# gau-nernst/llama-x

Measured on NVIDIA B200. Metric: train tokens/s, Llama-3.1-8B INT8+LoRA prefix-LM, higher is better.
Workload: dtype int8 fwd (int32 acc) / bf16 bwd

## Files before the change

include/llamax_b200.h:

```cpp
#ifndef LLAMAX_B200_H_
#define LLAMAX_B200_H_

#include <stdint.h>

#ifdef __cplusplus
extern "C" {
#endif

#define LLAMAX_B200_VERSION 102

#define LLAMAX_OK 0
#define LLAMAX_ERR_ARG (-1)
#define LLAMAX_ERR_CUDA (-2)

const char* llamax_last_error(void);
int llamax_version(void);
int llamax_set_device(int device);
int llamax_set_gemm_cta_group(int cg);

typedef struct {
  const void* lora_h;
  int64_t ldh;
  const void* lora_b;
  int32_t lora_rank;
  float lora_scale;
  const void* resid;
  int64_t ldr;
  int32_t seg_n0, seg_n1;
  const void* rope;
  int32_t rope_S, rope_cols;
} llamax_epilogue_t;

int llamax_int8_gemm_dequant(const void* A, int64_t lda, const void* B, int64_t ldb, const void* a_scale,
                             const void* b_scale, void* C, int64_t ldc, int64_t M, int64_t N, int64_t K,
                             const llamax_epilogue_t* epi, void* stream);
int llamax_int8_gemm_s32(const void* A, int64_t lda, const void* B, int64_t ldb, void* C, int64_t ldc, int64_t M,
                         int64_t N, int64_t K, void* stream);

int llamax_bf16_gemm(const void* A, int64_t lda, const void* B, int64_t ldb, void* C, int64_t ldc, int64_t M,
                     int64_t N, int64_t K, const void* col_scale, int round_before_scale,
                     const llamax_epilogue_t* epi, void* stream);
int llamax_bf16_gemm_swiglu_bwd(const void* A, int64_t lda, const void* B, int64_t ldb, int64_t M, int64_t N, int64_t K,
                                const llamax_epilogue_t* epi, const void* ab, int64_t ld_ab, void* dab, int64_t ld_dab,
                                void* g, void* stream);
int llamax_bf16_gemm_rowdot(const void* A, int64_t lda, const void* B, int64_t ldb, void* C, int64_t ldc, int64_t M,
                            int64_t N, int64_t K, const llamax_epilogue_t* epi, const void* other, int64_t ld_other,
                            void* dot_out, int64_t S, void* stream);

int llamax_bf16_int8_gemm(const void* A, int64_t lda, const void* B8, int64_t ldb8, const void* b_scale, int b_layout,
                          const void* tail, int64_t ldt, void* C, int64_t ldc, int64_t M, int64_t N, int64_t K,
                          int64_t K1, const llamax_epilogue_t* epi, void* stream);
int llamax_bf16_int8_gemm_swiglu_bwd(const void* A, int64_t lda, const void* B8, int64_t ldb8, const void* k_scale,
                                     int64_t M, int64_t N, int64_t K, const llamax_epilogue_t* epi, const void* ab,
                                     int64_t ld_ab, void* dab, int64_t ld_dab, void* g, void* stream);
int llamax_bf16_gemm_tn(const void* At, int64_t ldat, const void* Bt, int64_t ldbt, void* C, int64_t ldc, int64_t M,
                        int64_t N, int64_t K, void* stream);

int llamax_dequant_weight(const void* w8, const void* scale, void* out, int64_t ldo, int64_t N, int64_t K,
                          int transpose, int apply_scale, void* stream);

int llamax_rowquant_int8(const void* x, int64_t ldx, void* q8, void* scale_out, int64_t M, int64_t K,
                         void* stream);
int llamax_rowquant_int8_colscale(const void* x, int64_t ldx, const void* col_scale, void* q8, void* scale_out,
                                  int64_t M, int64_t K, void* stream);

int llamax_rmsnorm_fwd(const void* x, const void* w, void* y, void* rstd, void* q8, void* qscale, int64_t M,
                       int64_t D, float eps, void* stream);
int llamax_rmsnorm_bwd(const void* dy, const void* x, const void* w, const void* rstd, const void* dres, void* dx,
                       void* dw_partial, int32_t nparts, int64_t M, int64_t D, void* stream);
int llamax_reduce_partials(const void* partial, void* out, int32_t nparts, int64_t D, void* stream);

int llamax_swiglu_fwd(const void* a, const void* b, int64_t ld, void* g, void* q8, void* qscale, int64_t M,
                      int64_t F, void* stream);
int llamax_swiglu_bwd(const void* dg, const void* a, const void* b, int64_t ld, void* da, void* db, int64_t ldd,
                      void* g, int64_t M, int64_t F, void* stream);

int llamax_rope_inplace(void* x, int64_t ld, const void* rope, int64_t B, int64_t S, int32_t nheads, int32_t D,
                        int inverse, void* stream);

int llamax_attn_fwd(const void* q, int64_t ldq, const void* k, int64_t ldk, const void* v, int64_t ldv, void* o,
                    int64_t ldo, void* lse, int64_t B, int64_t S, int32_t Hq, int32_t Hkv, int32_t D,
                    int64_t prefix_len, const void* prefix_len_b, const void* doc_start, float scale, void* stream);
int llamax_attn_bwd(const void* q, int64_t ldq, const void* k, int64_t ldk, const void* v, int64_t ldv,
                    const void* o, int64_t ldo, const void* lse, const void* dout, int64_t lddo, void* dq,
                    int64_t lddq, void* dk, int64_t lddk, void* dv, int64_t lddv, void* dq_accum, void* delta,
                    int64_t B, int64_t S, int32_t Hq, int32_t Hkv, int32_t D, int64_t prefix_len,
                    const void* prefix_len_b, const void* doc_start, const void* doc_end, float scale,
                    const void* rope_inverse, void* stream);

int llamax_gelu_bias_fwd(void* z, const void* bias, void* y, int64_t rows, int64_t C, int32_t period, int32_t lo,
                         int32_t hi, void* stream);
int llamax_gelu_bwd(const void* dy, const void* z, void* dz, int64_t rows, int64_t C, int32_t period, int32_t lo,
                    int32_t hi, void* stream);
int llamax_conv_s2k3_col2im(const void* dcol, void* dxp, int64_t B, int64_t Tp, int64_t C, void* stream);

#define LLAMAX_MAX_COPY_JOBS 64
typedef struct {
  const void* src;
  void* dst;
  int64_t src_ld;
  int64_t dst_ld;
  int32_t rows, cols;
  float scale;
  int32_t flags;
} llamax_copy_job_t;
int llamax_batched_copy(const llamax_copy_job_t* jobs, int32_t n_jobs, void* stream);

int llamax_lora_wgrad(const void* X, int64_t ldx, const void* Ht, int64_t ldht, void* out, int64_t M, int64_t P,
                      int32_t R, float alpha, void* stream);

int llamax_lora_bwd_pair(const void* dY, int64_t lddy, const void* Bt, int64_t ldbt, const void* Ht, int64_t ldht,
                         void* dh, int64_t lddh, void* dht, int64_t lddht, void* dh_accum, void* dB, int64_t M,
                         int64_t N, int32_t R, float alpha, void* stream);


int llamax_cross_entropy(void* logits, int64_t ld, const void* labels, void* loss_sum, const void* inv_n, int64_t M,
                         int64_t V, int write_grad, void* stream);

#ifdef __cplusplus
}
#endif
#endif
```

llamax_b200/_lib.py:

```python

import ctypes
import os
import threading
from ctypes import POINTER, Structure, c_char_p, c_float, c_int, c_int32, c_int64, c_void_p

_HERE = os.path.dirname(os.path.abspath(__file__))
LIB_PATH = os.environ.get("LLAMAX_B200_LIB") or os.path.join(_HERE, "csrc", "libllamax_b200.so")

P = c_void_p
I64 = c_int64
I32 = c_int32


class Epilogue(Structure):

    _fields_ = [
        ("lora_h", P),
        ("ldh", I64),
        ("lora_b", P),
        ("lora_rank", I32),
        ("lora_scale", c_float),
        ("resid", P),
        ("ldr", I64),
        ("seg_n0", I32),
        ("seg_n1", I32),
        ("rope", P),
        ("rope_S", I32),
        ("rope_cols", I32),
    ]


EP = POINTER(Epilogue)

MAX_COPY_JOBS = 64


class CopyJob(Structure):

    _fields_ = [
        ("src", P),
        ("dst", P),
        ("src_ld", I64),
        ("dst_ld", I64),
        ("rows", I32),
        ("cols", I32),
        ("scale", c_float),
        ("flags", I32),
    ]

SIGNATURES = {
    "llamax_version": [],
    "llamax_set_device": [c_int],
    "llamax_set_gemm_cta_group": [c_int],
    "llamax_int8_gemm_dequant": [P, I64, P, I64, P, P, P, I64, I64, I64, I64, EP, P],
    "llamax_int8_gemm_s32": [P, I64, P, I64, P, I64, I64, I64, I64, P],
    "llamax_bf16_gemm": [P, I64, P, I64, P, I64, I64, I64, I64, P, c_int, EP, P],
    "llamax_bf16_gemm_swiglu_bwd": [P, I64, P, I64, I64, I64, I64, EP, P, I64, P, I64, P, P],
    "llamax_bf16_gemm_tn": [P, I64, P, I64, P, I64, I64, I64, I64, P],
    "llamax_bf16_gemm_rowdot": [P, I64, P, I64, P, I64, I64, I64, I64, EP, P, I64, P, I64, P],
    "llamax_bf16_int8_gemm": [P, I64, P, I64, P, c_int, P, I64, P, I64, I64, I64, I64, I64, EP, P],
    "llamax_bf16_int8_gemm_swiglu_bwd": [P, I64, P, I64, P, I64, I64, I64, EP, P, I64, P, I64, P, P],
    "llamax_dequant_weight": [P, P, P, I64, I64, I64, c_int, c_int, P],
    "llamax_rowquant_int8": [P, I64, P, P, I64, I64, P],
    "llamax_rowquant_int8_colscale": [P, I64, P, P, P, I64, I64, P],
    "llamax_rmsnorm_fwd": [P, P, P, P, P, P, I64, I64, c_float, P],
    "llamax_rmsnorm_bwd": [P, P, P, P, P, P, P, I32, I64, I64, P],
    "llamax_reduce_partials": [P, P, I32, I64, P],
    "llamax_swiglu_fwd": [P, P, I64, P, P, P, I64, I64, P],
    "llamax_swiglu_bwd": [P, P, P, I64, P, P, I64, P, I64, I64, P],
    "llamax_rope_inplace": [P, I64, P, I64, I64, I32, I32, c_int, P],
    "llamax_attn_fwd": [P, I64, P, I64, P, I64, P, I64, P, I64, I64, I32, I32, I32, I64, P, P, c_float, P],
    "llamax_attn_bwd": [P, I64, P, I64, P, I64, P, I64, P, P, I64, P, I64, P, I64, P, I64, P, P,
                        I64, I64, I32, I32, I32, I64, P, P, P, c_float, P, P],
    "llamax_lora_wgrad": [P, I64, P, I64, P, I64, I64, I32, c_float, P],
    "llamax_lora_bwd_pair": [P, I64, P, I64, P, I64, P, I64, P, I64, P, P, I64, I64, I32, c_float, P],
    "llamax_gelu_bias_fwd": [P, P, P, I64, I64, I32, I32, I32, P],
    "llamax_gelu_bwd": [P, P, P, I64, I64, I32, I32, I32, P],
    "llamax_conv_s2k3_col2im": [P, P, I64, I64, I64, P],
    "llamax_batched_copy": [POINTER(CopyJob), I32, P],
    "llamax_cross_entropy": [P, I64, P, P, P, I64, I64, c_int, P],
}

_lib = None
_lock = threading.Lock()


class LlamaxError(RuntimeError):
    pass


def load():
    global _lib
    if _lib is not None:
        return _lib
    with _lock:
        if _lib is not None:
            return _lib
        if not os.path.exists(LIB_PATH):
            raise LlamaxError(
                f"{LIB_PATH} not found: the CUDA extension is the only implementation of this path "
                "(no fallback). Build it with `python -m llamax_b200.build`."
            )
        lib = ctypes.CDLL(LIB_PATH)
        lib.llamax_last_error.restype = c_char_p
        lib.llamax_last_error.argtypes = []
        for name, argtypes in SIGNATURES.items():
            fn = getattr(lib, name)
            fn.restype = c_int
            fn.argtypes = argtypes
        _lib = lib
    return _lib


def check(rc: int, what: str):
    if rc != 0:
        msg = load().llamax_last_error().decode("utf-8", "replace")
        raise LlamaxError(f"{what} failed (code {rc}): {msg}")
```

llamax_b200/csrc/attention.cu:

```cuda
#include <type_traits>

#include "common.cuh"
#include "host_utils.h"
#include "llamax_b200.h"

namespace lx {

constexpr int kHD = 128;
constexpr float kLog2e = 1.4426950408889634f;
constexpr float kLn2 = 0.6931471805599453f;

__device__ __forceinline__ float ex2(float x) {
  float y;
  asm("ex2.approx.ftz.f32 %0, %1;" : "=f"(y) : "f"(x));
  return y;
}

#ifdef LX_ATTN_TRACE
__device__ long long* g_attn_trace = nullptr;
#define LX_TR(on, s, slot)                                                        \
  do {                                                                            \
    if ((on) && g_attn_trace && (s) < 128) g_attn_trace[(s) * 32 + (slot)] = clock64(); \
  } while (0)
#else
// ... 1423 lines not shown
            uint32_t v[32];
            tmem_ld_32x32(tO + c * 32, v);
            tmem_wait_ld();
#pragma unroll
            for (int e = 0; e < 32; ++e) v[e] = __float_as_uint(__uint_as_float(v[e]) * alpha);
            tmem_st_32x32(tO + c * 32, v);
          }
          tmem_wait_st();
        }
        if (x == 1 ? (i < n0) : (i > 0 && i - 1 < n1)) {
          mbar_wait(&xu_tok[(r & 1) * 2 + x], tokw[r & 1] & 1);
          ++tokw[r & 1];
        }
        float m_exp = (m_used == -INFINITY) ? 0.f : m_used;
        asm volatile("" : "+f"(m_exp));
        float rowsum = 0.f;
        uint32_t pc[2][16];
#pragma unroll
        for (int c = 0; c < 4; ++c) {
#pragma unroll
          for (int e = 0; e < 32; e += 2) {
            const float p0 = ex2(fmaf(__uint_as_float(sv[c][e]), p.scale_log2, -m_exp));
            const float p1 = ex2(fmaf(__uint_as_float(sv[c][e + 1]), p.scale_log2, -m_exp));
            rowsum += p0 + p1;
            pc[c & 1][e / 2] = pack_bf16(p0, p1);
          }
          if (c > 0) {
            tmem_wait_st();
            tc_fence_before();
            __syncwarp();
            if (lane_id() == 0) mbar_arrive(&p_chunk[x * 4 + c - 1]);
          }
          tmem_st_32x16(tS + c * 16, pc[c & 1]);
        }
        if (x == 0 ? (i < n1) : (i + 1 < n0)) {
          __syncwarp();
          if (lane_id() == 0) mbar_arrive(&xu_tok[(r & 1) * 2 + (x ^ 1)]);
        }
        tmem_wait_st();
        tc_fence_before();
        __syncwarp();
        if (lane_id() == 0) mbar_arrive(&p_chunk[x * 4 + 3]);
        l = l * alpha + rowsum;
      }
      if (n_kv > 0) {
        mbar_wait(&pv_done[x], (sc - 1) & 1);
        tc_fence_after();
        const float inv_l = 1.f / l;
        const bool row_ok = q < p.S;
        __nv_bfloat16* orow = p.o + ((int64_t)it.b * p.S + q) * p.ldo + (int64_t)it.h * kD;
#pragma unroll 1
        for (int c = 0; c < kD / 32; ++c) {
          uint32_t v[32];
          tmem_ld_32x32(tO + c * 32, v);
          tmem_wait_ld();
          if (row_ok) {
#pragma unroll
            for (int e = 0; e < 32; e += 8) {
              uint4 o4;
              o4.x = pack_bf16(__uint_as_float(v[e]) * inv_l, __uint_as_float(v[e + 1]) * inv_l);
              o4.y = pack_bf16(__uint_as_float(v[e + 2]) * inv_l, __uint_as_float(v[e + 3]) * inv_l);
              o4.z = pack_bf16(__uint_as_float(v[e + 4]) * inv_l, __uint_as_float(v[e + 5]) * inv_l);
              o4.w = pack_bf16(__uint_as_float(v[e + 6]) * inv_l, __uint_as_float(v[e + 7]) * inv_l);
              stg_v4(orow + c * 32 + e, o4);
            }
          }
        }
        if (row_ok) p.lse[((int64_t)it.b * p.Hq + it.h) * p.S + q] = (m_used + log2f(l)) * kLn2;
        tc_fence_before();
      }
    }
    tc_fence_before();
  }

  tc_fence_before();
  __syncthreads();
  if (warp == 3) tmem_dealloc<1>(tmem_base, 512);
}

struct AttnBwdParams {
  const float* lse;
  const float* delta;
  float* dq_accum;
  __nv_bfloat16* dk;
  int64_t lddk;
  __nv_bfloat16* dv;
  int64_t lddv;
  int B, S, Hq, Hkv, P;
  int D;
  float scale, scale_log2;
  const int32_t* doc_start;
  const int32_t* doc_end;
  const float* rope;
  const int32_t* prefix_b;
};

namespace bwd {
constexpr int kKV = 128;
constexpr int kQ = 128;
constexpr int kThreads = 512;
constexpr int kWorkers = 256;
constexpr int kRegsCtrl = 64, kRegsWork = 144, kRegsDrain = 160;
constexpr int kTileBytes = 128 * kHD * 2;
constexpr int kOffK = 0;
constexpr int kOffV = kOffK + kTileBytes;
constexpr int kOffQ = kOffV + kTileBytes;
constexpr int kOffdO = kOffQ + 2 * kTileBytes;
constexpr int kOffdS = kOffdO + kTileBytes;
constexpr int kOffdQ = kOffdS + kTileBytes;
constexpr int kStageRows = 32;
constexpr int kdQBytes = kStageRows * kHD * 4;
constexpr int kOffStat = kOffdQ + kdQBytes;
constexpr int kOffBar = kOffStat + 2 * 3 * kQ * 4;
constexpr int kNumBars = 1 + 4 + 2 + 4 + 2 + 1;
constexpr int kSmemBytes = kOffBar + kNumBars * 8 + 16 + 1024;
static_assert(kSmemBytes <= 232448, "attention backward shared memory budget");
constexpr int kColdV = 0, kColdK = 128, kColX = 256, kColY = 384;
}

template <bool kDocs, int kD>
__global__ void __launch_bounds__(bwd::kThreads, 1)
attn_bwd_kernel(const __grid_constant__ CUtensorMap tmQ, const __grid_constant__ CUtensorMap tmK,
                const __grid_constant__ CUtensorMap tmV, const __grid_constant__ CUtensorMap tmdO,
                const AttnBwdParams p) {
  using namespace bwd;
  extern __shared__ uint8_t smem_raw[];
  uint8_t* smem = reinterpret_cast<uint8_t*>((reinterpret_cast<uintptr_t>(smem_raw) + 1023) & ~uintptr_t(1023));
  float* s_stat = reinterpret_cast<float*>(smem + kOffStat);
  uint64_t* bars = reinterpret_cast<uint64_t*>(smem + kOffBar);
  uint64_t* kv_full = bars;
  uint64_t* q_full = bars + 1;
  uint64_t* q_empty = bars + 3;
  uint64_t* do_full = bars + 5;
  uint64_t* do_empty = bars + 6;
  uint64_t* s_full = bars + 7;
  uint64_t* p_full = bars + 8;
  uint64_t* dp_full = bars + 9;
  uint64_t* ds_full = bars + 10;
  uint64_t* dq_full = bars + 11;
  uint64_t* dq_empty = bars + 12;
  uint64_t* acc_done = bars + 13;
  uint32_t* tmem_slot = reinterpret_cast<uint32_t*>(bars + kNumBars);

  const int warp = threadIdx.x >> 5;
  const int hk = blockIdx.x, jt = blockIdx.y, b = blockIdx.z;
  const int Pb = p.prefix_b ? min(max(p.prefix_b[b], 0), p.S) : p.P;
#ifdef LX_ATTN_TRACE
  const bool tr_cta = (blockIdx.x | blockIdx.y | blockIdx.z) == 0 && (threadIdx.x & 31) == 0 &&
                      (warp == 1 || warp == 4 || warp == 12);
#endif
  const int kv0 = jt * kKV;
  const int G = p.Hq / p.Hkv;
  const int nq_tiles = (p.S + kQ - 1) / kQ;
  const int i_start = (kv0 < Pb) ? 0 : kv0 / kQ;
  const int i_end = kDocs ? min(nq_tiles, p.doc_end[(int64_t)b * p.S + min(kv0 + kKV - 1, p.S - 1)] / kQ + 1) : nq_tiles;
  const int steps_per_head = i_end - i_start;
  const int n_steps = G * steps_per_head;

  if (warp == 0 && elect_one()) {
    tma_prefetch_desc(&tmQ);
    tma_prefetch_desc(&tmK);
    tma_prefetch_desc(&tmV);
    tma_prefetch_desc(&tmdO);
  }
  if (warp == 1 && elect_one()) {
    mbar_init(kv_full, 1);
    for (int i = 0; i < 2; ++i) {
      mbar_init(&q_full[i], 1);
      mbar_init(&q_empty[i], 1);
    }
    mbar_init(do_full, 1);
    mbar_init(do_empty, 1);
    mbar_init(s_full, 1);
    mbar_init(p_full, 8);
    mbar_init(dp_full, 1);
    mbar_init(ds_full, 8);
    mbar_init(dq_full, 1);
    mbar_init(dq_empty, 4);
    mbar_init(acc_done, 1);
    fence_mbar_init();
  }
  if (warp == 2) {
    tmem_alloc<1>(tmem_slot, 512);
    tmem_relinquish<1>();
  }
  tc_fence_before();
  __syncthreads();
  tc_fence_after();
  const uint32_t tmem_base = *tmem_slot;

  if (warp < 4) {
    setmaxnreg_dec<kRegsCtrl>();
    if (warp == 0) {
      if (elect_one()) {
        mbar_expect_tx(kv_full, 2 * kTileBytes);
        tma_load_4d(smem + kOffK, &tmK, kv_full, 0, hk, kv0, b);
        tma_load_4d(smem + kOffK + kTileBytes / 2, &tmK, kv_full, 64, hk, kv0, b);
        tma_load_4d(smem + kOffV, &tmV, kv_full, 0, hk, kv0, b);
        tma_load_4d(smem + kOffV + kTileBytes / 2, &tmV, kv_full, 64, hk, kv0, b);
        for (int s = 0; s < n_steps; ++s) {
          const int st = s & 1;
          const int hq = hk * G + s / steps_per_head;
          const int q0 = (i_start + s % steps_per_head) * kQ;
          mbar_wait(&q_empty[st], ((s >> 1) & 1) ^ 1);
          mbar_expect_tx(&q_full[st], kTileBytes);
          uint8_t* sq = smem + kOffQ + st * kTileBytes;
          tma_load_4d(sq, &tmQ, &q_full[st], 0, hq, q0, b);
          tma_load_4d(sq + kTileBytes / 2, &tmQ, &q_full[st], 64, hq, q0, b);
          mbar_wait(do_empty, (s & 1) ^ 1);
          mbar_expect_tx(do_full, kTileBytes);
          uint8_t* sdo = smem + kOffdO;
          tma_load_4d(sdo, &tmdO, do_full, 0, hq, q0, b);
          tma_load_4d(sdo + kTileBytes / 2, &tmdO, do_full, 64, hq, q0, b);
        }
      }
      __syncwarp();
    } else if (warp == 1) {
      if (elect_one()) {
        constexpr uint32_t idesc_st = make_idesc(1, 1, 128, 128, 0, 0);
        constexpr uint32_t idesc_acc = make_idesc(1, 1, 128, 128, 0, 1);
        constexpr uint32_t idesc_dq = make_idesc(1, 1, 128, 128, 1, 1);
        constexpr uint32_t kHi = desc_hi(1024);
        const uint32_t loK = desc_lo(smem_u32(smem + kOffK), 16), loV = desc_lo(smem_u32(smem + kOffV), 16);
        const uint32_t loKmn = desc_lo(smem_u32(smem + kOffK), 16384);
        const uint32_t loQ0 = desc_lo(smem_u32(smem + kOffQ), 16), loQmn0 = desc_lo(smem_u32(smem + kOffQ), 16384);
        const uint32_t lodO = desc_lo(smem_u32(smem + kOffdO), 16), lodOmn = desc_lo(smem_u32(smem + kOffdO), 16384);
        const uint32_t lodS = desc_lo(smem_u32(smem + kOffdS), 16), lodSmn = desc_lo(smem_u32(smem + kOffdS), 16384);
        const uint32_t tX = tmem_base + kColX, tY = tmem_base + kColY;
        auto mma_kk = [&](uint32_t d, uint32_t a_lo, uint32_t b_lo) {
#pragma unroll
          for (int dh = 0; dh < 2; ++dh)
#pragma unroll
            for (int ks = 0; ks < 4; ++ks)
              umma_ss<false, 1>(d, desc_join(a_lo + (dh * 16384 + ks * 32) / 16, kHi),
                                desc_join(b_lo + (dh * 16384 + ks * 32) / 16, kHi), idesc_st, (dh | ks) != 0);
        };
        mbar_wait(kv_full, 0);
        mbar_wait(&q_full[0], 0);
// ... 143 lines not shown
            }
        };
        if (full_tile) block(std::false_type{});
        else block(std::true_type{});
      }
      tmem_st_32x32(tXw, pr);
      tmem_wait_st();
      tc_fence_before();
      __syncwarp();
      if (lane_id() == 0) mbar_arrive(p_full);
      LX_TR(tr_cta, s, 9);

      mbar_wait(dp_full, s & 1);
      tc_fence_after();
      LX_TR(tr_cta, s, 10);
#pragma unroll
      for (int c = 0; c < 2; ++c) {
        uint32_t dv[32], dsr[16];
        tmem_ld_32x32(tYw + c * 32, dv);
        tmem_wait_ld_regs(dv);
#pragma unroll
        for (int i = 0; i < 32; i += 4) {
          const float4 d4 = lds_f4(stat_u + kQ * 4 + (c * 32 + i) * 4);
          const uint32_t p01 = pr[c * 16 + i / 2], p23 = pr[c * 16 + i / 2 + 1];
          const float ds0 = bf16_lo(p01) * fmaf(__uint_as_float(dv[i]), p.scale, -d4.x);
          const float ds1 = bf16_hi(p01) * fmaf(__uint_as_float(dv[i + 1]), p.scale, -d4.y);
          const float ds2 = bf16_lo(p23) * fmaf(__uint_as_float(dv[i + 2]), p.scale, -d4.z);
          const float ds3 = bf16_hi(p23) * fmaf(__uint_as_float(dv[i + 3]), p.scale, -d4.w);
          dsr[i / 2] = pack_bf16(ds0, ds1);
          dsr[i / 2 + 1] = pack_bf16(ds2, ds3);
        }
#pragma unroll
        for (int cc = 0; cc < 4; ++cc)
          sts_v4(sdS + (((c * 4 + cc) ^ (t & 7)) << 4), dsr[cc * 4], dsr[cc * 4 + 1], dsr[cc * 4 + 2], dsr[cc * 4 + 3]);
      }
      fence_proxy_async_smem();
      tc_fence_before();
      __syncwarp();
      if (lane_id() == 0) mbar_arrive(ds_full);
      LX_TR(tr_cta, s, 11);
      store_stat(st ^ 1, nxt_a, nxt_d);
    }
    mbar_wait(acc_done, 0);
    tc_fence_after();
    const bool row_ok = kv < p.S;
    __nv_bfloat16* drow = grp == 0 ? p.dv + ((int64_t)b * p.S + kv) * p.lddv + (int64_t)hk * kD
                                   : p.dk + ((int64_t)b * p.S + kv) * p.lddk + (int64_t)hk * kD;
#pragma unroll 1
    for (int c = 0; c < kD / 32; ++c) {
      uint32_t v[32];
      tmem_ld_32x32(tmem_base + (grp == 0 ? kColdV : kColdK) + lane_off + c * 32, v);
      tmem_wait_ld_regs(v);
      if (row_ok && grp == 1 && p.rope != nullptr) {
        const float4* cs = reinterpret_cast<const float4*>(p.rope + ((int64_t)kv * (kD / 2) + c * 16) * 2);
#pragma unroll
        for (int i = 0; i < 32; i += 4) {
          const float4 t4 = cs[i / 4];
          const float g0 = __uint_as_float(v[i]), g1 = __uint_as_float(v[i + 1]);
          const float g2 = __uint_as_float(v[i + 2]), g3 = __uint_as_float(v[i + 3]);
          v[i] = __float_as_uint(g0 * t4.x + g1 * t4.y);
          v[i + 1] = __float_as_uint(g1 * t4.x - g0 * t4.y);
          v[i + 2] = __float_as_uint(g2 * t4.z + g3 * t4.w);
          v[i + 3] = __float_as_uint(g3 * t4.z - g2 * t4.w);
        }
      }
      if (row_ok) {
#pragma unroll
        for (int i = 0; i < 32; i += 8) {
          uint4 o4;
          o4.x = pack_bf16(__uint_as_float(v[i]), __uint_as_float(v[i + 1]));
          o4.y = pack_bf16(__uint_as_float(v[i + 2]), __uint_as_float(v[i + 3]));
          o4.z = pack_bf16(__uint_as_float(v[i + 4]), __uint_as_float(v[i + 5]));
          o4.w = pack_bf16(__uint_as_float(v[i + 6]), __uint_as_float(v[i + 7]));
          stg_v4(drow + c * 32 + i, o4);
        }
      }
    }
    tc_fence_before();
  } else {
    setmaxnreg_inc<kRegsDrain>();
    const int lq = warp & 3;
    const int t = lq * 32 + lane_id();
    const uint32_t lane_off = uint32_t(lq * 32) << 16;
    for (int s = 0; s < n_steps; ++s) {
      const int hq = hk * G + s / steps_per_head;
      const int q0 = (i_start + s % steps_per_head) * kQ;
      LX_TR(tr_cta, s, 12);
      mbar_wait(dq_full, s & 1);
      tc_fence_after();
      LX_TR(tr_cta, s, 13);
      uint32_t v[4][32];
#pragma unroll
      for (int r = 0; r < 4; ++r) tmem_ld_32x32(tmem_base + kColY + r * 32 + lane_off, v[r]);
#pragma unroll
      for (int r = 0; r < 4; ++r) tmem_wait_ld_regs(v[r]);
      tc_fence_before();
      __syncwarp();
      if (lane_id() == 0) mbar_arrive(dq_empty);
      LX_TR(tr_cta, s, 14);
      if (t < kD) {
        float* dst = p.dq_accum + (((int64_t)b * p.Hq + hq) * p.S + q0) * kD + t;
        const int rows = min(kQ, p.S - q0);
#pragma unroll
        for (int r = 0; r < 4; ++r)
#pragma unroll
          for (int i = 0; i < 32; ++i)
            if (r * 32 + i < rows) red_add_f32(dst + (r * 32 + i) * kD, __uint_as_float(v[r][i]));
      }
      LX_TR(tr_cta, s, 15);
    }
  }

  tc_fence_before();
  __syncthreads();
  if (warp == 2) tmem_dealloc<1>(tmem_base, 512);
}

template <int D>
__global__ void __launch_bounds__(256) attn_delta_kernel(const __nv_bfloat16* __restrict__ o, int64_t ldo,
                                                         const __nv_bfloat16* __restrict__ dout, int64_t lddo,
                                                         float* __restrict__ delta, int S, int Hq) {
  constexpr int kLanes = D / 8;
  constexpr int kHeadsPerWarp = 32 / kLanes;
  const int lane = threadIdx.x & 31;
  const int grp = blockIdx.y * 8 + (threadIdx.x >> 5);
  const int h = grp * kHeadsPerWarp + lane / kLanes;
  if (grp * kHeadsPerWarp >= Hq) return;
  const int64_t row = blockIdx.x;
  float s = 0.f;
  if (h < Hq) {
    const int c = h * D + (lane % kLanes) * 8;
    const uint4 a = ldg_nc_v4(o + row * ldo + c);
    const uint4 g = ldg_nc_v4(dout + row * lddo + c);
    s = bf16_lo(a.x) * bf16_lo(g.x) + bf16_hi(a.x) * bf16_hi(g.x) + bf16_lo(a.y) * bf16_lo(g.y) +
        bf16_hi(a.y) * bf16_hi(g.y) + bf16_lo(a.z) * bf16_lo(g.z) + bf16_hi(a.z) * bf16_hi(g.z) +
        bf16_lo(a.w) * bf16_lo(g.w) + bf16_hi(a.w) * bf16_hi(g.w);
  }
#pragma unroll
  for (int off = kLanes / 2; off > 0; off >>= 1) s += __shfl_xor_sync(0xffffffffu, s, off);
  if (h < Hq && (lane % kLanes) == 0) {
    const unsigned bb = blockIdx.x / (unsigned)S, ss = blockIdx.x - bb * (unsigned)S;
    delta[((int64_t)bb * Hq + h) * S + ss] = s;
  }
}

template <int D>
__global__ void __launch_bounds__(256) attn_dq_convert_kernel(const float* __restrict__ acc,
                                                              __nv_bfloat16* __restrict__ dq, int64_t lddq, int S,
                                                              int Hq, const float* __restrict__ rope) {
  constexpr int kVecs = D / 8;
  const unsigned bh = blockIdx.x, b = bh / (unsigned)Hq, h = bh - b * (unsigned)Hq;
  const float* slab = acc + (int64_t)bh * S * D;
  const int nvec = S * kVecs;
  float4 lo[2], hi[2], t0[2], t1[2];
  int t[2];
#pragma unroll
  for (int k = 0; k < 2; ++k) {
    t[k] = blockIdx.y * 512 + k * 256 + threadIdx.x;
    if (t[k] < nvec) {
      const float* src = slab + (int64_t)t[k] * 8;
      lo[k] = __ldcs(reinterpret_cast<const float4*>(src));
      hi[k] = __ldcs(reinterpret_cast<const float4*>(src + 4));
      if (rope != nullptr) {
        const int s_ = t[k] / kVecs, c = (t[k] % kVecs) * 8;
        const float4* cs = reinterpret_cast<const float4*>(rope + ((int64_t)s_ * (D / 2) + c / 2) * 2);
        t0[k] = __ldg(cs);
        t1[k] = __ldg(cs + 1);
      }
    }
  }
#pragma unroll
  for (int k = 0; k < 2; ++k) {
    if (t[k] >= nvec) continue;
    const int s_ = t[k] / kVecs, c = (t[k] % kVecs) * 8;
    float4 a = lo[k], b4 = hi[k];
    if (rope != nullptr) {
      const float4 u0 = t0[k], u1 = t1[k];
      a = make_float4(a.x * u0.x + a.y * u0.y, a.y * u0.x - a.x * u0.y, a.z * u0.z + a.w * u0.w, a.w * u0.z - a.z * u0.w);
      b4 = make_float4(b4.x * u1.x + b4.y * u1.y, b4.y * u1.x - b4.x * u1.y, b4.z * u1.z + b4.w * u1.w,
                       b4.w * u1.z - b4.z * u1.w);
    }
    uint4 o4;
    o4.x = pack_bf16(a.x, a.y);
    o4.y = pack_bf16(a.z, a.w);
    o4.z = pack_bf16(b4.x, b4.y);
    o4.w = pack_bf16(b4.z, b4.w);
    *reinterpret_cast<uint4*>(dq + ((int64_t)b * S + s_) * lddq + (int64_t)h * D + c) = o4;
  }
}

static int make_head_tmap(CUtensorMap* m, const void* ptr, int64_t ld, int64_t B, int64_t S, int H, int D,
                          int box_rows) {
  const int64_t dims[4] = {D, H, S, B};
  const int64_t strides[3] = {D, ld, S * ld};
  const int box[4] = {64, 1, box_rows, 1};
  return make_tmap_4d(m, CU_TENSOR_MAP_DATA_TYPE_BFLOAT16, 2, ptr, dims, strides, box);
}

static int check_attn_args(int64_t B, int64_t S, int Hq, int Hkv, int D, int64_t P, const char* who) {
  if (D != 128 && D != 64) return set_error(LLAMAX_ERR_ARG, "attention: head_dim must be 64 or 128");
  if (B <= 0 || S <= 0 || Hq <= 0 || Hkv <= 0 || Hq % Hkv) return set_error(LLAMAX_ERR_ARG, "attention: bad B/S/H");
  if (P < 0) return set_error(LLAMAX_ERR_ARG, "attention: prefix_len < 0");
  if (B * S > 0x7fffffffLL || B * Hq > 0x7fffffffLL || S * 16 > 0x7fffffffLL)
    return set_error(LLAMAX_ERR_ARG, "attention: B * S, B * Hq and 16 * S must be below 2^31");
  (void)who;
  return 0;
}

}

using namespace lx;

extern "C" {

#ifdef LX_ATTN_TRACE
int llamax_debug_attn_trace(void* buf) {
  long long* b = (long long*)buf;
  cudaError_t e = cudaMemcpyToSymbol(g_attn_trace, &b, sizeof(b));
  return e == cudaSuccess ? 0 : set_cuda_error(e, "debug_attn_trace");
}
#endif

int llamax_attn_fwd(const void* q, int64_t ldq, const void* k, int64_t ldk, const void* v, int64_t ldv, void* o,
                    int64_t ldo, void* lse, int64_t B, int64_t S, int32_t Hq, int32_t Hkv, int32_t D,
                    int64_t prefix_len, const void* prefix_len_b, const void* doc_start, float scale, void* stream) {
  if (!q || !k || !v || !o || !lse) return set_error(LLAMAX_ERR_ARG, "attn_fwd: null pointer");
  int rc = check_attn_args(B, S, Hq, Hkv, D, prefix_len, "attn_fwd");
  if (rc) return rc;
  if (ldq % 8 || ldk % 8 || ldv % 8 || ldo % 8) return set_error(LLAMAX_ERR_ARG, "attn_fwd: pitches must be multiples of 8");
  CUtensorMap tq, tk, tv;
  if ((rc = make_head_tmap(&tq, q, ldq, B, S, Hq, D, fwd::kTile))) return rc;
  if ((rc = make_head_tmap(&tk, k, ldk, B, S, Hkv, D, fwd::kTile))) return rc;
  if ((rc = make_head_tmap(&tv, v, ldv, B, S, Hkv, D, fwd::kTile))) return rc;
  static const int version = [] {
    const char* e = getenv("LLAMAX_ATTN_FWD");
    if (getenv("LLAMAX_ATTN_FWD_ONE_TILE") && getenv("LLAMAX_ATTN_FWD_ONE_TILE")[0] == '1') return 1;
    return (e != nullptr && e[0] >= '1' && e[0] <= '5') ? e[0] - '0' : 5;
  }();
  const int version_eff = (version >= 4 && doc_start != nullptr) ? 2 : version;
  if (version_eff == 5) {
    auto kern5 = D == 128 ? attn_fwd5_kernel<128> : attn_fwd5_kernel<64>;
    if ((rc = ensure_dyn_smem(reinterpret_cast<const void*>(kern5), fwd5::kSmemBytes5, "attn_fwd: cudaFuncSetAttribute"))) return rc;
    AttnFwdParams p5;
    p5.o = (__nv_bfloat16*)o;
    p5.ldo = ldo;
    p5.lse = (float*)lse;
    p5.B = (int)B; p5.S = (int)S; p5.Hq = Hq; p5.Hkv = Hkv;
    p5.P = (int)std::min<int64_t>(prefix_len, S);
    p5.D = D;
    p5.scale_log2 = scale * kLog2e;
    p5.doc_start = nullptr;
    p5.prefix_b = (const int32_t*)prefix_len_b;
    const int n_pairs = (int)((ceil_div(S, fwd::kTile) + 1) / 2);
    const int64_t n_items = (int64_t)n_pairs * B * Hq;
    const int grid5 = (int)std::min<int64_t>(n_items, sm_count());
    kern5<<<grid5, fwd4::kThreads, fwd5::kSmemBytes5, (cudaStream_t)stream>>>(tq, tk, tv, p5, n_pairs);
    LX_CHECK_LAUNCH("attn_fwd");
    return 0;
  }
  const bool one_tile = version_eff == 1;
  auto kern1 = doc_start ? (D == 128 ? attn_fwd_kernel<true, 128> : attn_fwd_kernel<true, 64>)
                         : (D == 128 ? attn_fwd_kernel<false, 128> : attn_fwd_kernel<false, 64>);
  auto kern2 = doc_start ? (D == 128 ? attn_fwd2_kernel<true, 128> : attn_fwd2_kernel<true, 64>)
                         : (D == 128 ? attn_fwd2_kernel<false, 128> : attn_fwd2_kernel<false, 64>);
  auto kern3 = doc_start ? (D == 128 ? attn_fwd3_kernel<true, 128> : attn_fwd3_kernel<true, 64>)
                         : (D == 128 ? attn_fwd3_kernel<false, 128> : attn_fwd3_kernel<false, 64>);
  static const bool alu_pack = getenv("LLAMAX_ATTN_ALU_PACK") && getenv("LLAMAX_ATTN_ALU_PACK")[0] == '1';
  static const bool stagger = !(getenv("LLAMAX_ATTN_STAGGER") && getenv("LLAMAX_ATTN_STAGGER")[0] == '0');
  auto pick4 = [&](auto docs_tag, auto d_tag) {
    constexpr bool kDc = decltype(docs_tag)::value;
    constexpr int kDd = decltype(d_tag)::value;
    return alu_pack ? (stagger ? attn_fwd4_kernel<kDc, kDd, true, true> : attn_fwd4_kernel<kDc, kDd, true, false>)
                    : (stagger ? attn_fwd4_kernel<kDc, kDd, false, true> : attn_fwd4_kernel<kDc, kDd, false, false>);
  };
  auto kern4 = doc_start ? (D == 128 ? pick4(std::true_type{}, std::integral_constant<int, 128>{})
                                     : pick4(std::true_type{}, std::integral_constant<int, 64>{}))
                         : (D == 128 ? pick4(std::false_type{}, std::integral_constant<int, 128>{})
                                     : pick4(std::false_type{}, std::integral_constant<int, 64>{}));
  auto kern = version_eff == 1 ? kern1 : version_eff == 2 ? kern2 : version_eff == 3 ? kern3 : kern4;
  const int smem_bytes = version_eff == 1 ? fwd::smem_bytes(fwd::kNB) : version_eff == 2 ? fwd2::kSmemBytes
                         : version_eff == 3 ? fwd3::kSmemBytes : fwd4::kSmemBytes;
  const int threads = version_eff == 1 ? fwd::kThreads : version_eff == 2 ? fwd2::kThreads
                      : version_eff == 3 ? fwd3::kThreads : fwd4::kThreads;
  if ((rc = ensure_dyn_smem(reinterpret_cast<const void*>(kern), smem_bytes, "attn_fwd: cudaFuncSetAttribute"))) return rc;
  AttnFwdParams p;
  p.o = (__nv_bfloat16*)o;
  p.ldo = ldo;
  p.lse = (float*)lse;
  p.B = (int)B; p.S = (int)S; p.Hq = Hq; p.Hkv = Hkv;
  p.P = (int)std::min<int64_t>(prefix_len, S);
  p.D = D;
  p.scale_log2 = scale * kLog2e;
  p.doc_start = (const int32_t*)doc_start;
  p.prefix_b = (const int32_t*)prefix_len_b;
  const unsigned q_tiles = (unsigned)ceil_div(S, fwd::kTile);
  dim3 grid(Hq, (unsigned)B, one_tile ? q_tiles : (q_tiles + 1) / 2);
  kern<<<grid, threads, smem_bytes, (cudaStream_t)stream>>>(tq, tk, tv, p);
  LX_CHECK_LAUNCH("attn_fwd");
  return 0;
}

int llamax_attn_bwd(const void* q, int64_t ldq, const void* k, int64_t ldk, const void* v, int64_t ldv,
                    const void* o, int64_t ldo, const void* lse, const void* dout, int64_t lddo, void* dq,
                    int64_t lddq, void* dk, int64_t lddk, void* dv, int64_t lddv, void* dq_accum, void* delta,
                    int64_t B, int64_t S, int32_t Hq, int32_t Hkv, int32_t D, int64_t prefix_len,
                    const void* prefix_len_b, const void* doc_start, const void* doc_end, float scale,
                    const void* rope_inverse, void* stream) {
  if ((doc_start == nullptr) != (doc_end == nullptr))
    return set_error(LLAMAX_ERR_ARG, "attn_bwd: doc_start and doc_end go together");
  if (!q || !k || !v || !lse || !dout || !dq || !dk || !dv || !dq_accum || !delta)
    return set_error(LLAMAX_ERR_ARG, "attn_bwd: null pointer");
  int rc = check_attn_args(B, S, Hq, Hkv, D, prefix_len, "attn_bwd");
  if (rc) return rc;
  if (ldq % 8 || ldk % 8 || ldv % 8 || (o != nullptr && ldo % 8) || lddo % 8 || lddq % 8 || lddk % 8 || lddv % 8)
    return set_error(LLAMAX_ERR_ARG, "attn_bwd: pitches must be multiples of 8");
  cudaStream_t st = (cudaStream_t)stream;
  const int64_t rows = B * S;
  cudaError_t e = cudaMemsetAsync(dq_accum, 0, (size_t)rows * Hq * D * sizeof(float), st);
  if (e != cudaSuccess) return set_cuda_error(e, "attn_bwd: memset");
  if (o != nullptr) {
    const int groups = (int)ceil_div(Hq, 32 / (D / 8));
    dim3 dgrid((unsigned)rows, (unsigned)ceil_div(groups, 8));
    if (D == 128)
      attn_delta_kernel<128><<<dgrid, 256, 0, st>>>((const __nv_bfloat16*)o, ldo, (const __nv_bfloat16*)dout, lddo,
                                                    (float*)delta, (int)S, Hq);
    else
      attn_delta_kernel<64><<<dgrid, 256, 0, st>>>((const __nv_bfloat16*)o, ldo, (const __nv_bfloat16*)dout, lddo,
                                                   (float*)delta, (int)S, Hq);
    LX_CHECK_LAUNCH("attn_bwd: delta");
  }
  CUtensorMap tq, tk, tv, tdo;
  if ((rc = make_head_tmap(&tq, q, ldq, B, S, Hq, D, bwd::kQ))) return rc;
  if ((rc = make_head_tmap(&tdo, dout, lddo, B, S, Hq, D, bwd::kQ))) return rc;
  if ((rc = make_head_tmap(&tk, k, ldk, B, S, Hkv, D, bwd::kKV))) return rc;
  if ((rc = make_head_tmap(&tv, v, ldv, B, S, Hkv, D, bwd::kKV))) return rc;
  auto kern = doc_start ? (D == 128 ? attn_bwd_kernel<true, 128> : attn_bwd_kernel<true, 64>)
                        : (D == 128 ? attn_bwd_kernel<false, 128> : attn_bwd_kernel<false, 64>);
  if ((rc = ensure_dyn_smem(reinterpret_cast<const void*>(kern), bwd::kSmemBytes, "attn_bwd: cudaFuncSetAttribute"))) return rc;
  AttnBwdParams p;
  p.lse = (const float*)lse;
  p.delta = (const float*)delta;
  p.dq_accum = (float*)dq_accum;
  p.dk = (__nv_bfloat16*)dk; p.lddk = lddk;
  p.dv = (__nv_bfloat16*)dv; p.lddv = lddv;
  p.B = (int)B; p.S = (int)S; p.Hq = Hq; p.Hkv = Hkv;
  p.P = (int)std::min<int64_t>(prefix_len, S);
  p.D = D;
  p.scale = scale;
  p.scale_log2 = scale * kLog2e;
  p.doc_start = (const int32_t*)doc_start;
  p.doc_end = (const int32_t*)doc_end;
  p.rope = (const float*)rope_inverse;
  p.prefix_b = (const int32_t*)prefix_len_b;
  dim3 grid(Hkv, (unsigned)ceil_div(S, bwd::kKV), (unsigned)B);
  kern<<<grid, bwd::kThreads, bwd::kSmemBytes, st>>>(tq, tk, tv, tdo, p);
  LX_CHECK_LAUNCH("attn_bwd");
  {
    dim3 cgrid((unsigned)(B * Hq), (unsigned)ceil_div(S * (D / 8), 512));
    if (D == 128)
      attn_dq_convert_kernel<128><<<cgrid, 256, 0, st>>>((const float*)dq_accum, (__nv_bfloat16*)dq, lddq, (int)S, Hq,
                                                          (const float*)rope_inverse);
    else
      attn_dq_convert_kernel<64><<<cgrid, 256, 0, st>>>((const float*)dq_accum, (__nv_bfloat16*)dq, lddq, (int)S, Hq,
                                                         (const float*)rope_inverse);
    LX_CHECK_LAUNCH("attn_bwd: dq convert");
  }
  return 0;
}

}
```

llamax_b200/ops.py:

```python

import ctypes
import threading

import torch
from torch import Tensor

from . import _lib
from ._lib import Epilogue, check

_tls = threading.local()


class _KernelTiming:

    def __init__(self):
        self.on = False
        self.only = None
        self.records = []

    def enable(self, only=None):
        self.records, self.on, self.only = [], True, (set(only) if only else None)

    def disable(self):
        self.on = False
# ... 451 lines not shown
    lib, st = _prep(dcol)
    assert dcol.dtype is torch.bfloat16 and dcol.is_contiguous() and dcol.shape == (B * (Tp // 2), 3 * C)
    dxp = torch.empty(B, Tp, C, device=dcol.device, dtype=torch.bfloat16)
    _call(lib, "llamax_conv_s2k3_col2im", (_p(dcol), _p(dxp), B, Tp, C, st), "col2im", 0.0, 5.0 * B * Tp * C)
    return dxp


def batched_copy(jobs) -> None:
    jobs = list(jobs)
    if not jobs:
        return
    lib, st = _prep(jobs[0][0])
    for i0 in range(0, len(jobs), _lib.MAX_COPY_JOBS):
        chunk = jobs[i0 : i0 + _lib.MAX_COPY_JOBS]
        arr = (_lib.CopyJob * len(chunk))()
        for k, (src, dst, scale, transpose) in enumerate(chunk):
            assert src.dim() == 2 and dst.dim() == 2 and src.stride(1) == 1 and dst.stride(1) == 1
            assert dst.dtype is torch.bfloat16 and src.dtype in (torch.bfloat16, torch.float32)
            assert tuple(dst.shape) == ((src.shape[1], src.shape[0]) if transpose else tuple(src.shape))
            j = arr[k]
            j.src, j.dst = src.data_ptr(), dst.data_ptr()
            j.src_ld, j.dst_ld = src.stride(0), dst.stride(0)
            j.rows, j.cols = src.shape
            j.scale = float(scale)
            j.flags = (1 if src.dtype is torch.float32 else 0) | (2 if transpose else 0)
        _call(lib, "llamax_batched_copy", (arr, len(chunk), st), "batched_copy", 0.0, 0.0)


def cross_entropy_(logits: Tensor, labels: Tensor, loss_sum: Tensor, inv_n: Tensor | None, write_grad: bool):
    lib, st = _prep(logits)
    assert logits.dtype is torch.bfloat16 and logits.dim() == 2 and logits.stride(1) == 1
    assert labels.dtype is torch.int64 and labels.is_contiguous() and labels.numel() == logits.shape[0]
    assert loss_sum.dtype is torch.float32 and (inv_n is None or inv_n.dtype is torch.float32)
    M, V = logits.shape
    _call(lib, "llamax_cross_entropy",
          (_p(logits), logits.stride(0), _p(labels), _p(loss_sum), _p(inv_n), M, V, int(write_grad), st),
          "cross_entropy", 0.0, (4.0 if write_grad else 2.0) * M * V)


def _pairs(S: int, prefix_len) -> float:
    if isinstance(prefix_len, Tensor):
        if not TIMING.on:
            return 0.0
        return float(sum(_pairs(S, int(v)) for v in prefix_len.tolist())) / max(1, prefix_len.numel())
    P_ = min(int(prefix_len), S)
    return S * P_ + (S - P_) * (S - P_ + 1) / 2


def _prefix_args(prefix_len, B: int, device):
    if isinstance(prefix_len, Tensor):
        pb = prefix_len.to(device=device, dtype=torch.int32).reshape(-1).contiguous()
        assert pb.numel() == B, f"per-sequence prefix_len must have {B} entries"
        return 0, pb
    return int(prefix_len), None


def doc_bounds(doc_ids: Tensor):
    B, S = doc_ids.shape
    idx = torch.arange(S, device=doc_ids.device).expand(B, S)
    first = torch.ones_like(doc_ids, dtype=torch.bool)
    first[:, 1:] = doc_ids[:, 1:] != doc_ids[:, :-1]
    last = torch.ones_like(first)
    last[:, :-1] = first[:, 1:]
    start = torch.where(first, idx, torch.zeros_like(idx)).cummax(dim=1).values
    end = torch.where(last, idx, torch.full_like(idx, S - 1)).flip(1).cummin(dim=1).values.flip(1)
    return start.to(torch.int32).contiguous(), end.to(torch.int32).contiguous()


def attn_fwd(q: Tensor, k: Tensor, v: Tensor, B: int, S: int, Hq: int, Hkv: int, D: int, prefix_len,
             scale: float | None = None, doc_start: Tensor | None = None):
    lib, st = _prep(q)
    for t in (q, k, v):
        assert t.dtype is torch.bfloat16 and t.dim() == 2 and t.stride(1) == 1 and t.shape[0] == B * S
    o = torch.empty(B * S, Hq * D, device=q.device, dtype=torch.bfloat16)
    lse = torch.empty(B, Hq, S, device=q.device, dtype=torch.float32)
    scale = float(scale) if scale is not None else D ** -0.5
    p_scalar, p_b = _prefix_args(prefix_len, B, q.device)
    _call(lib, "llamax_attn_fwd",
          (_p(q), q.stride(0), _p(k), k.stride(0), _p(v), v.stride(0), _p(o), o.stride(0), _p(lse), B, S, Hq, Hkv, D, p_scalar, _p(p_b), _p(doc_start), scale, st,),
          "attn_fwd", 4.0 * B * Hq * D * _pairs(S, prefix_len), 0.0)
    return o, lse


def attn_bwd(q, k, v, o, lse, dout, dq, dk, dv, B, S, Hq, Hkv, D, prefix_len, scale=None, doc_start=None,
             doc_end=None, rope_inverse=None, delta=None):
    if rope_inverse is not None:
        assert rope_inverse.dtype is torch.float32 and rope_inverse.is_contiguous()
        assert rope_inverse.shape[0] >= S and rope_inverse.shape[1] == D // 2
    lib, st = _prep(q)
    dout = _rows(dout)
    dq_accum = torch.empty(B * S, Hq * D, device=q.device, dtype=torch.float32)
    if delta is None:
        delta = torch.empty(B, Hq, S, device=q.device, dtype=torch.float32)
    else:
        assert delta.dtype is torch.float32 and delta.shape == (B, Hq, S) and delta.is_contiguous()
        o = None
    scale = float(scale) if scale is not None else D ** -0.5
    p_scalar, p_b = _prefix_args(prefix_len, B, q.device)
    _call(lib, "llamax_attn_bwd",
          (_p(q), q.stride(0), _p(k), k.stride(0), _p(v), v.stride(0), _p(o), o.stride(0) if o is not None else 0, _p(lse), _p(dout), dout.stride(0), _p(dq), dq.stride(0), _p(dk), dk.stride(0), _p(dv), dv.stride(0), _p(dq_accum), _p(delta), B, S, Hq, Hkv, D, p_scalar, _p(p_b), _p(doc_start), _p(doc_end), scale, _p(rope_inverse), st,),
          "attn_bwd", 10.0 * B * Hq * D * _pairs(S, prefix_len), 0.0)
    return dq, dk, dv
```

Baseline: 43280.

## Fuse dQ conversion into attention backward via per-tile completion counters

Drops the separate memset of the fp32 dQ accumulator and the follow-up dq-convert kernel. Each q-tile gets an atomic arrival counter; the last KV block CTA to add into a tile applies inverse RoPE, writes bf16 dQ, and re-zeroes the accumulator and counter so a persistent workspace stays clean across calls. This saves a full write pass and a read pass of the fp32 accumulator plus one kernel launch. In exchange the dQ warps in every step pay a fence, two barriers and an atomic, and correctness depends on the contributor count matching the actual producers.

```diff
diff --git a/include/llamax_b200.h b/include/llamax_b200.h
--- a/include/llamax_b200.h
+++ b/include/llamax_b200.h
@@ -87,6 +87,7 @@
                     int64_t B, int64_t S, int32_t Hq, int32_t Hkv, int32_t D, int64_t prefix_len,
                     const void* prefix_len_b, const void* doc_start, const void* doc_end, float scale,
                     const void* rope_inverse, void* stream);
+int llamax_attn_bwd_workspace_bytes(int64_t B, int64_t S, int32_t Hq, int32_t D, int64_t* bytes);
 
 int llamax_gelu_bias_fwd(void* z, const void* bias, void* y, int64_t rows, int64_t C, int32_t period, int32_t lo,
                          int32_t hi, void* stream);
diff --git a/llamax_b200/_lib.py b/llamax_b200/_lib.py
--- a/llamax_b200/_lib.py
+++ b/llamax_b200/_lib.py
@@ -72,6 +72,7 @@
     "llamax_attn_fwd": [P, I64, P, I64, P, I64, P, I64, P, I64, I64, I32, I32, I32, I64, P, P, c_float, P],
     "llamax_attn_bwd": [P, I64, P, I64, P, I64, P, I64, P, P, I64, P, I64, P, I64, P, I64, P, P,
                         I64, I64, I32, I32, I32, I64, P, P, P, c_float, P, P],
+    "llamax_attn_bwd_workspace_bytes": [I64, I64, I32, I32, POINTER(I64)],
     "llamax_lora_wgrad": [P, I64, P, I64, P, I64, I64, I32, c_float, P],
     "llamax_lora_bwd_pair": [P, I64, P, I64, P, I64, P, I64, P, I64, P, P, I64, I64, I32, c_float, P],
     "llamax_gelu_bias_fwd": [P, P, P, I64, I64, I32, I32, I32, P],
diff --git a/llamax_b200/csrc/attention.cu b/llamax_b200/csrc/attention.cu
--- a/llamax_b200/csrc/attention.cu
+++ b/llamax_b200/csrc/attention.cu
@@ -1529,6 +1529,9 @@
   const float* lse;
   const float* delta;
   float* dq_accum;
+  uint32_t* dq_count;
+  __nv_bfloat16* dq;
+  int64_t lddq;
   __nv_bfloat16* dk;
   int64_t lddk;
   __nv_bfloat16* dv;
@@ -1554,15 +1557,88 @@
 constexpr int kOffQ = kOffV + kTileBytes;
 constexpr int kOffdO = kOffQ + 2 * kTileBytes;
 constexpr int kOffdS = kOffdO + kTileBytes;
-constexpr int kOffdQ = kOffdS + kTileBytes;
-constexpr int kStageRows = 32;
-constexpr int kdQBytes = kStageRows * kHD * 4;
-constexpr int kOffStat = kOffdQ + kdQBytes;
+constexpr int kOffStat = kOffdS + kTileBytes;
 constexpr int kOffBar = kOffStat + 2 * 3 * kQ * 4;
 constexpr int kNumBars = 1 + 4 + 2 + 4 + 2 + 1;
 constexpr int kSmemBytes = kOffBar + kNumBars * 8 + 16 + 1024;
 static_assert(kSmemBytes <= 232448, "attention backward shared memory budget");
 constexpr int kColdV = 0, kColdK = 128, kColX = 256, kColY = 384;
+constexpr int kFinishBatch = 4;
+}
+
+template <bool kDocs>
+__device__ __forceinline__ int2 bwd_q_tiles(const AttnBwdParams& p, int b, int Pb, int jt, int nq_tiles) {
+  const int kv0 = jt * bwd::kKV;
+  const int i_start = (kv0 < Pb) ? 0 : kv0 / bwd::kQ;
+  const int i_end = kDocs ? min(nq_tiles, p.doc_end[(int64_t)b * p.S + min(kv0 + bwd::kKV - 1, p.S - 1)] / bwd::kQ + 1)
+                          : nq_tiles;
+  return make_int2(i_start, i_end);
+}
+
+template <bool kDocs>
+__device__ int bwd_dq_contributors(const AttnBwdParams& p, int b, int Pb, int i, int nq_tiles) {
+  int n = 0;
+#pragma unroll 4
+  for (int jt = 0; jt < nq_tiles; ++jt) {
+    const int2 r = bwd_q_tiles<kDocs>(p, b, Pb, jt, nq_tiles);
+    n += (r.x <= i && i < r.y) ? 1 : 0;
+  }
+  return n;
+}
+
+__device__ __forceinline__ uint4 dq_finish8(float4 a, float4 b4, const float* rope, int D, int pos, int c) {
+  if (rope != nullptr) {
+    const float4* cs = reinterpret_cast<const float4*>(rope + ((int64_t)pos * (D / 2) + c / 2) * 2);
+    const float4 u0 = __ldg(cs), u1 = __ldg(cs + 1);
+    a = make_float4(a.x * u0.x + a.y * u0.y, a.y * u0.x - a.x * u0.y, a.z * u0.z + a.w * u0.w, a.w * u0.z - a.z * u0.w);
+    b4 = make_float4(b4.x * u1.x + b4.y * u1.y, b4.y * u1.x - b4.x * u1.y, b4.z * u1.z + b4.w * u1.w,
+                     b4.w * u1.z - b4.z * u1.w);
+  }
+  uint4 o4;
+  o4.x = pack_bf16(a.x, a.y);
+  o4.y = pack_bf16(a.z, a.w);
+  o4.z = pack_bf16(b4.x, b4.y);
+  o4.w = pack_bf16(b4.z, b4.w);
+  return o4;
+}
+
+template <int kD>
+__device__ __forceinline__ void bwd_dq_finish(const AttnBwdParams& p, int b, int hq, int q0, int rows, int t) {
+  constexpr int kVecs = kD / 8;
+  constexpr int kB = bwd::kFinishBatch;
+  float* tile = p.dq_accum + (((int64_t)b * p.Hq + hq) * p.S + q0) * kD;
+  const int nvec = rows * kVecs;
+  const float4 zero = make_float4(0.f, 0.f, 0.f, 0.f);
+#pragma unroll 1
+  for (int v0 = 0; v0 < nvec; v0 += 128 * kB) {
+    float4 lo[kB], hi[kB];
+#pragma unroll
+    for (int k = 0; k < kB; ++k) {
+      const int v = v0 + k * 128 + t;
+      lo[k] = hi[k] = zero;
+      if (v < nvec) {
+        lo[k] = __ldcg(reinterpret_cast<const float4*>(tile + (int64_t)v * 8));
+        hi[k] = __ldcg(reinterpret_cast<const float4*>(tile + (int64_t)v * 8 + 4));
+      }
+    }
+#pragma unroll
+    for (int k = 0; k < kB; ++k) {
+      const int v = v0 + k * 128 + t;
+      if (v < nvec) {
+        const int pos = q0 + v / kVecs, c = (v % kVecs) * 8;
+        *reinterpret_cast<uint4*>(p.dq + ((int64_t)b * p.S + pos) * p.lddq + (int64_t)hq * kD + c) =
+            dq_finish8(lo[k], hi[k], p.rope, kD, pos, c);
+        *reinterpret_cast<float4*>(tile + (int64_t)v * 8) = zero;
+        *reinterpret_cast<float4*>(tile + (int64_t)v * 8 + 4) = zero;
+      }
+    }
+  }
+}
+
+__device__ __forceinline__ uint32_t atom_add_acq_rel_gpu(uint32_t* p, uint32_t v) {
+  uint32_t old;
+  asm volatile("atom.acq_rel.gpu.global.add.u32 %0, [%1], %2;" : "=r"(old) : "l"(p), "r"(v) : "memory");
+  return old;
 }
 
 template <bool kDocs, int kD>
@@ -1599,8 +1675,8 @@
   const int kv0 = jt * kKV;
   const int G = p.Hq / p.Hkv;
   const int nq_tiles = (p.S + kQ - 1) / kQ;
-  const int i_start = (kv0 < Pb) ? 0 : kv0 / kQ;
-  const int i_end = kDocs ? min(nq_tiles, p.doc_end[(int64_t)b * p.S + min(kv0 + kKV - 1, p.S - 1)] / kQ + 1) : nq_tiles;
+  const int2 q_tiles = bwd_q_tiles<kDocs>(p, b, Pb, jt, nq_tiles);
+  const int i_start = q_tiles.x, i_end = q_tiles.y;
   const int steps_per_head = i_end - i_start;
   const int n_steps = G * steps_per_head;
 
@@ -1910,9 +1986,13 @@
     const int lq = warp & 3;
     const int t = lq * 32 + lane_id();
     const uint32_t lane_off = uint32_t(lq * 32) << 16;
+    volatile uint32_t* s_finish = tmem_slot + 1;
     for (int s = 0; s < n_steps; ++s) {
       const int hq = hk * G + s / steps_per_head;
-      const int q0 = (i_start + s % steps_per_head) * kQ;
+      const int i = i_start + s % steps_per_head;
+      const int q0 = i * kQ;
+      const int rows = min(kQ, p.S - q0);
+      const int expected = t == 0 ? bwd_dq_contributors<kDocs>(p, b, Pb, i, nq_tiles) : 0;
       LX_TR(tr_cta, s, 12);
       mbar_wait(dq_full, s & 1);
       tc_fence_after();
@@ -1928,12 +2008,21 @@
       LX_TR(tr_cta, s, 14);
       if (t < kD) {
         float* dst = p.dq_accum + (((int64_t)b * p.Hq + hq) * p.S + q0) * kD + t;
-        const int rows = min(kQ, p.S - q0);
 #pragma unroll
         for (int r = 0; r < 4; ++r)
 #pragma unroll
-          for (int i = 0; i < 32; ++i)
-            if (r * 32 + i < rows) red_add_f32(dst + (r * 32 + i) * kD, __uint_as_float(v[r][i]));
+          for (int e = 0; e < 32; ++e)
+            if (r * 32 + e < rows) red_add_f32(dst + (r * 32 + e) * kD, __uint_as_float(v[r][e]));
+      }
+      __threadfence();
+      named_bar_sync(2, 128);
+      uint32_t* cnt = p.dq_count + ((int64_t)b * p.Hq + hq) * nq_tiles + i;
+      if (t == 0) *s_finish = (atom_add_acq_rel_gpu(cnt, 1) + 1 == (uint32_t)expected) ? 1u : 0u;
+      named_bar_sync(2, 128);
+      if (*s_finish) {
+        __threadfence();
+        bwd_dq_finish<kD>(p, b, hq, q0, rows, t);
+        if (t == 0) *cnt = 0;
       }
       LX_TR(tr_cta, s, 15);
     }
@@ -1972,51 +2061,6 @@
   }
 }
 
-template <int D>
-__global__ void __launch_bounds__(256) attn_dq_convert_kernel(const float* __restrict__ acc,
-                                                              __nv_bfloat16* __restrict__ dq, int64_t lddq, int S,
-                                                              int Hq, const float* __restrict__ rope) {
-  constexpr int kVecs = D / 8;
-  const unsigned bh = blockIdx.x, b = bh / (unsigned)Hq, h = bh - b * (unsigned)Hq;
-  const float* slab = acc + (int64_t)bh * S * D;
-  const int nvec = S * kVecs;
-  float4 lo[2], hi[2], t0[2], t1[2];
-  int t[2];
-#pragma unroll
-  for (int k = 0; k < 2; ++k) {
-    t[k] = blockIdx.y * 512 + k * 256 + threadIdx.x;
-    if (t[k] < nvec) {
-      const float* src = slab + (int64_t)t[k] * 8;
-      lo[k] = __ldcs(reinterpret_cast<const float4*>(src));
-      hi[k] = __ldcs(reinterpret_cast<const float4*>(src + 4));
-      if (rope != nullptr) {
-        const int s_ = t[k] / kVecs, c = (t[k] % kVecs) * 8;
-        const float4* cs = reinterpret_cast<const float4*>(rope + ((int64_t)s_ * (D / 2) + c / 2) * 2);
-        t0[k] = __ldg(cs);
-        t1[k] = __ldg(cs + 1);
-      }
-    }
-  }
-#pragma unroll
-  for (int k = 0; k < 2; ++k) {
-    if (t[k] >= nvec) continue;
-    const int s_ = t[k] / kVecs, c = (t[k] % kVecs) * 8;
-    float4 a = lo[k], b4 = hi[k];
-    if (rope != nullptr) {
-      const float4 u0 = t0[k], u1 = t1[k];
-      a = make_float4(a.x * u0.x + a.y * u0.y, a.y * u0.x - a.x * u0.y, a.z * u0.z + a.w * u0.w, a.w * u0.z - a.z * u0.w);
-      b4 = make_float4(b4.x * u1.x + b4.y * u1.y, b4.y * u1.x - b4.x * u1.y, b4.z * u1.z + b4.w * u1.w,
-                       b4.w * u1.z - b4.z * u1.w);
-    }
-    uint4 o4;
-    o4.x = pack_bf16(a.x, a.y);
-    o4.y = pack_bf16(a.z, a.w);
-    o4.z = pack_bf16(b4.x, b4.y);
-    o4.w = pack_bf16(b4.z, b4.w);
-    *reinterpret_cast<uint4*>(dq + ((int64_t)b * S + s_) * lddq + (int64_t)h * D + c) = o4;
-  }
-}
-
 static int make_head_tmap(CUtensorMap* m, const void* ptr, int64_t ld, int64_t B, int64_t S, int H, int D,
                           int box_rows) {
   const int64_t dims[4] = {D, H, S, B};
@@ -2033,6 +2077,11 @@
     return set_error(LLAMAX_ERR_ARG, "attention: B * S, B * Hq and 16 * S must be below 2^31");
   (void)who;
   return 0;
+}
+
+static int64_t attn_bwd_accum_bytes(int64_t B, int64_t S, int Hq, int D) { return B * Hq * S * D * (int64_t)sizeof(float); }
+static int64_t attn_bwd_workspace_size(int64_t B, int64_t S, int Hq, int D) {
+  return attn_bwd_accum_bytes(B, S, Hq, D) + B * Hq * ceil_div(S, bwd::kQ) * (int64_t)sizeof(uint32_t);
 }
 
 }
@@ -2144,8 +2193,6 @@
     return set_error(LLAMAX_ERR_ARG, "attn_bwd: pitches must be multiples of 8");
   cudaStream_t st = (cudaStream_t)stream;
   const int64_t rows = B * S;
-  cudaError_t e = cudaMemsetAsync(dq_accum, 0, (size_t)rows * Hq * D * sizeof(float), st);
-  if (e != cudaSuccess) return set_cuda_error(e, "attn_bwd: memset");
   if (o != nullptr) {
     const int groups = (int)ceil_div(Hq, 32 / (D / 8));
     dim3 dgrid((unsigned)rows, (unsigned)ceil_div(groups, 8));
@@ -2169,6 +2216,8 @@
   p.lse = (const float*)lse;
   p.delta = (const float*)delta;
   p.dq_accum = (float*)dq_accum;
+  p.dq_count = reinterpret_cast<uint32_t*>(static_cast<char*>(dq_accum) + attn_bwd_accum_bytes(B, S, Hq, D));
+  p.dq = (__nv_bfloat16*)dq; p.lddq = lddq;
   p.dk = (__nv_bfloat16*)dk; p.lddk = lddk;
   p.dv = (__nv_bfloat16*)dv; p.lddv = lddv;
   p.B = (int)B; p.S = (int)S; p.Hq = Hq; p.Hkv = Hkv;
@@ -2183,17 +2232,15 @@
   dim3 grid(Hkv, (unsigned)ceil_div(S, bwd::kKV), (unsigned)B);
   kern<<<grid, bwd::kThreads, bwd::kSmemBytes, st>>>(tq, tk, tv, tdo, p);
   LX_CHECK_LAUNCH("attn_bwd");
-  {
-    dim3 cgrid((unsigned)(B * Hq), (unsigned)ceil_div(S * (D / 8), 512));
-    if (D == 128)
-      attn_dq_convert_kernel<128><<<cgrid, 256, 0, st>>>((const float*)dq_accum, (__nv_bfloat16*)dq, lddq, (int)S, Hq,
-                                                          (const float*)rope_inverse);
-    else
-      attn_dq_convert_kernel<64><<<cgrid, 256, 0, st>>>((const float*)dq_accum, (__nv_bfloat16*)dq, lddq, (int)S, Hq,
-                                                         (const float*)rope_inverse);
-    LX_CHECK_LAUNCH("attn_bwd: dq convert");
-  }
   return 0;
 }
 
-}
+int llamax_attn_bwd_workspace_bytes(int64_t B, int64_t S, int32_t Hq, int32_t D, int64_t* bytes) {
+  if (bytes == nullptr) return set_error(LLAMAX_ERR_ARG, "attn_bwd_workspace_bytes: null pointer");
+  int rc = check_attn_args(B, S, Hq, 1, D, 0, "attn_bwd_workspace_bytes");
+  if (rc) return rc;
+  *bytes = attn_bwd_workspace_size(B, S, Hq, D);
+  return 0;
+}
+
+}
diff --git a/llamax_b200/ops.py b/llamax_b200/ops.py
--- a/llamax_b200/ops.py
+++ b/llamax_b200/ops.py
@@ -557,6 +557,22 @@
     return o, lse
 
 
+_ATTN_BWD_WORKSPACE: dict = {}
+
+
+def attn_bwd_workspace(lib, device: torch.device, B: int, S: int, Hq: int, D: int) -> Tensor:
+    n = ctypes.c_int64()
+    check(lib.llamax_attn_bwd_workspace_bytes(B, S, Hq, D, ctypes.byref(n)), "llamax_attn_bwd_workspace_bytes")
+    idx = device.index if device.index is not None else torch.cuda.current_device()
+    ws = _ATTN_BWD_WORKSPACE.get(idx)
+    if ws is None or ws.numel() < n.value:
+        if torch.cuda.is_current_stream_capturing():
+            raise _lib.LlamaxError("attn_bwd: workspace would be allocated during graph capture; call once before")
+        ws = torch.zeros(n.value, device=device, dtype=torch.uint8)
+        _ATTN_BWD_WORKSPACE[idx] = ws
+    return ws
+
+
 def attn_bwd(q, k, v, o, lse, dout, dq, dk, dv, B, S, Hq, Hkv, D, prefix_len, scale=None, doc_start=None,
              doc_end=None, rope_inverse=None, delta=None):
     if rope_inverse is not None:
@@ -564,7 +580,7 @@
         assert rope_inverse.shape[0] >= S and rope_inverse.shape[1] == D // 2
     lib, st = _prep(q)
     dout = _rows(dout)
-    dq_accum = torch.empty(B * S, Hq * D, device=q.device, dtype=torch.float32)
+    dq_accum = attn_bwd_workspace(lib, q.device, B, S, Hq, D)
     if delta is None:
         delta = torch.empty(B, Hq, S, device=q.device, dtype=torch.float32)
     else:
```

Result: slower. 40860, median of 6 (-5.6%).
